# NVIDIA-Genomics-Research/GenomeWorks

Measured on AMD Instinct MI355X. Metric: cudapoa consensus GCUPS, 1024-window short-read batch (static band 256, 32 reads <= 1024 bp), higher is better.
Workload: dtype int16; 1 GPU; BASELINE configs[2]: cudapoa single-batch consensus, 1024 windows x 32 reads, backbone 960 bp, <=48 sub/24 ins/24 del, BatchConfig(1024,32,256,static_band), scores 8/-6/-8; windows_per_gpu=1024, cells_per_gpu=10990578176, parallelism=index-split x1

## Files before the change

### genomeworks_amd/csrc/gwhip_poa.hip

```cpp
#include <hip/hip_runtime.h>

#include <cstdio>
#include <cstdlib>
#include <cstring>
#include <string>

#include "poa_device.h"
#include "poa_full_device.h"
#include "poa_graph_device.h"
#include "poa_tb_device.h"

namespace gwhip
{

#ifndef GWHIP_POA_PART
thread_local std::string g_last_error;

static int fail(hipError_t e, const char* what)
{
    g_last_error = std::string(what) + ": " + hipGetErrorString(e);
    return (int)e;
}
static int fail_msg(int code, const std::string& msg)
{
    g_last_error = msg;
    return code;
}
#endif

constexpr int kRingBytes   = 8448;
constexpr int kRowInfoLds  = 3074;
constexpr int kRowInfoBytes = kRowInfoLds * 8;
constexpr int kReadLds     = 2048;
constexpr int kCodeTileLds = 4096;
static_assert(kReadLds + kCodeTileLds >= 3072 * 2, "the incremental topsort keeps the previous order (uint16 x 3072) in the read + code-tile regions");
constexpr int kBsRingBytes   = 2048;
constexpr int kReadWinBytes  = 4096;
constexpr int kMwLds         = 768;
constexpr size_t kReservedCuLds = 128 * 1024;

struct KernelArgs
{
    gwhip_poa_config cfg;
    PoaLayout L;
    int32_t total_windows;
    const uint8_t* sequences;
    const int8_t* base_weights;
    int32_t* sequence_lengths;
    const gwhip_window_details* window_details;
    uint8_t* consensus;
    uint16_t* coverage;
    uint8_t* msa;
    uint8_t* workspace;
    uint8_t* full_scores;
    uint64_t* cells;
    uint64_t* phase_cycles;
    int32_t debug_flags;
    int32_t cons_lds_nodes;
    int32_t wide_ring_bytes;
    uint32_t* work_counters;
};

// ... 2 lines not shown
{
    GraphView<IdT> g;
    g.nodes                = slab + L.nodes;
    g.incoming_edge_count  = (uint16_t*)(slab + L.in_cnt);
    g.outgoing_edge_count  = (uint16_t*)(slab + L.out_cnt);
    g.node_alignment_count = (uint16_t*)(slab + L.aln_cnt);
    g.coverage             = (uint16_t*)(slab + L.coverage);
    g.sorted_poa           = (IdT*)(slab + L.sorted);
    g.node_id_to_pos       = (IdT*)(slab + L.pos);
    g.local_cnt            = (uint16_t*)(slab + L.local_cnt);
    g.incoming_edges       = (IdT*)(slab + L.in_edges);
    g.incoming_edge_w      = (uint16_t*)(slab + L.in_w);
    g.outgoing_edges       = (IdT*)(slab + L.out_edges);
    g.node_alignments      = (IdT*)(slab + L.aligned);
    g.cons_scores          = (int32_t*)(slab + L.cons_scores);
    g.cons_pred            = (IdT*)(slab + L.cons_pred);
    g.marks                = slab + L.marks;
    g.check                = slab + L.check;
    g.to_visit             = (IdT*)(slab + L.to_visit);
    g.out_cov              = (uint16_t*)(slab + L.out_cov);
    g.out_cov_cnt          = (uint16_t*)(slab + L.out_cov_cnt);
    g.msa_pos              = (IdT*)(slab + L.msa_pos);
    g.seq_begin            = (IdT*)(slab + L.seq_begin);
    return g;
}

template <typename ScoreT, typename IdT, typename TraceT, int BM, bool MSA, bool LDS_TABLES, int NW, int VARIANT>
__global__ __launch_bounds__(kWave * NW) void poa_window_kernel(KernelArgs a)
{
    constexpr bool DBG = VARIANT == 1 || VARIANT == 4 || VARIANT == 6;
    constexpr int PV   = VARIANT == 0 ? 0 : (VARIANT <= 2 ? 1 : 2);
    constexpr bool kFullPacked = (VARIANT == 5 || VARIANT == 6) && BM == GWHIP_FULL_BAND && LDS_TABLES && std::is_same<ScoreT, int16_t>::value;
    const int32_t debug_flags = DBG ? a.debug_flags : 0;
    extern __shared__ __attribute__((aligned(16))) uint8_t smem[];
    const int lane       = threadIdx.x & (kWave - 1);
    const int wave       = __builtin_amdgcn_readfirstlane((int)threadIdx.x >> 6);
    for (int32_t w = blockIdx.x; w < a.total_windows;)
    {
    const gwhip_poa_config& c = a.cfg;
    uint8_t* slab        = a.workspace + (size_t)w * a.L.per_window;
    GraphView<IdT> g     = carve_graph<IdT>(slab, a.L);
    const gwhip_window_details wd = a.window_details[w];
    int32_t* seq_lens    = a.sequence_lengths + wd.seq_len_buffer_offset;
    const uint8_t* sequence    = a.sequences + wd.seq_starts;
    const int8_t* base_weights = a.base_weights + wd.seq_starts;
    uint8_t* consensus   = a.consensus + (size_t)w * c.max_consensus_size;
    int32_t* alignment_graph = (int32_t*)(slab + a.L.align_graph);
    int32_t* alignment_read  = (int32_t*)(slab + a.L.align_read);

    ScoreT* ring = reinterpret_cast<ScoreT*>(smem);
    uint8_t* lds_rowinfo_region = smem + kRingBytes;
    uint8_t* lds_read_buf       = smem + kRingBytes + kRowInfoBytes;
    uint8_t* lds_code_tile      = LDS_TABLES ? smem + kRingBytes + kRowInfoBytes + kReadLds : nullptr;
    const int32_t ring_bytes    = LDS_TABLES ? kRingBytes : a.wide_ring_bytes;
    int32_t* lds_bs_ring        = LDS_TABLES ? nullptr : reinterpret_cast<int32_t*>(smem + ring_bytes);
    uint8_t* lds_read_window    = LDS_TABLES ? nullptr : smem + ring_bytes + kBsRingBytes;
    uint8_t* codes              = a.L.codes ? slab + a.L.codes : nullptr;
    constexpr bool graph_fits_lds = LDS_TABLES;
    using RowT = RowInfo<LDS_TABLES>;
    RowT* rowinfo;
    if constexpr (LDS_TABLES)
        rowinfo = reinterpret_cast<RowT*>(smem + kRingBytes);
    else
        rowinfo = reinterpret_cast<RowT*>(slab + a.L.rowinfo);

    constexpr bool TB = (BM == GWHIP_STATIC_BAND_TRACEBACK || BM == GWHIP_ADAPTIVE_BAND_TRACEBACK);
    ScoreT* scores;
    uint8_t* full_moves = nullptr;
    if (BM == GWHIP_FULL_BAND)
    {
        const size_t cell_bytes = sizeof(ScoreT) + (sizeof(ScoreT) == 2 ? 1 : 0);
        uint8_t* region         = a.full_scores + (size_t)wd.scores_offset * (size_t)c.max_nodes_per_graph * cell_bytes;
        scores                  = reinterpret_cast<ScoreT*>(region);
        if (sizeof(ScoreT) == 2) full_moves = region + (size_t)wd.scores_width * (size_t)c.max_nodes_per_graph * sizeof(ScoreT);
    }
    else
        scores = reinterpret_cast<ScoreT*>(slab + a.L.scores);
    TraceT* traceback = TB ? reinterpret_cast<TraceT*>(slab + a.L.trace) : nullptr;
    const float banded_buffer_size = __fmul_rn((float)c.max_nodes_per_graph, (float)c.matrix_sequence_dimension);
    MwArgs<ScoreT>* mw_args = nullptr;
    MwShared* mw_shared     = nullptr;
    if constexpr (NW > 1)
    {
        {
            int32_t bases = lane < (int32_t)wd.num_seqs ? seq_lens[lane] : 0;
            for (int off = 32; off > 0; off >>= 1) bases += __shfl_xor(bases, off);
            bases = __builtin_amdgcn_readfirstlane(bases);
// ... 7 lines not shown
        mw_shared = reinterpret_cast<MwShared*>(smem + ring_bytes + kBsRingBytes + kReadWinBytes + 128);
        if (wave != 0)
        {
            for (;;)
            {
                block_barrier();
                const MwArgs<ScoreT> A = *mw_args;
                if (A.op != 1) return;
                generic_forward_skew<ScoreT, IdT, RowT, DBG>(A, g, rowinfo, ring, mw_shared, wave, lane);
            }
        }
    }

    const int32_t len0 = seq_lens[0];
    for (int32_t i = lane; i < len0; i += kWave)
    {
        g.nodes[i]                = sequence[i];
        g.sorted_poa[i]           = (IdT)i;
        g.node_id_to_pos[i]       = (IdT)i;
        g.node_alignment_count[i] = 0;
        g.coverage[i]             = 1;
        g.outgoing_edge_count[i]  = (i == len0 - 1) ? 0 : 1;
        g.local_cnt[i] = (uint16_t)(1 | ((i == len0 - 1 ? 0 : 1) << 4) | ((i == 0 ? 0 : 1) << 10));
        if (i < len0 - 1)
        {
            g.outgoing_edges[(int64_t)i * kEdges] = (IdT)(i + 1);
            if (MSA)
            {
                g.out_cov[(int64_t)i * kEdges * c.max_sequences_per_poa] = 0;
                g.out_cov_cnt[(int64_t)i * kEdges]                       = 1;
            }
        }
        if (i == 0)
        {
            g.incoming_edge_count[0] = 0;
            g.incoming_edge_w[0]     = (uint16_t)base_weights[0];
            if (MSA) g.seq_begin[0] = 0;
        }
        else
        {
            g.incoming_edges[(int64_t)i * kEdges]  = (IdT)(i - 1);
            g.incoming_edge_w[(int64_t)i * kEdges] = (uint16_t)(base_weights[i - 1] + base_weights[i]);
            g.incoming_edge_count[i]               = 1;
        }
    }
    if (lane == 0) consensus[0] = 0;
    uint64_t cells = 0;
    int32_t node_count = len0;
    uint64_t phase_acc[kPhCount] = {0, 0, 0, 0, 0, 0};
    PhaseClock pc{(DBG && a.phase_cycles) ? phase_acc : nullptr, 0};
    wave_sync();
    pc.start();

    for (int32_t s = 1; s < (int32_t)wd.num_seqs; s++)
    {
        const int32_t seq_len = seq_lens[s];
        const int32_t adv     = ((s == 1 ? len0 : seq_lens[s - 1]) + 3) & ~3;
        sequence += adv;
        base_weights += adv;

        if (node_count >= c.max_nodes_per_graph)
        {
            if (lane == 0) { consensus[0] = kKernelError; consensus[1] = kNodeCountExceeded; }
            break;
        }
        pc.tick(kPhOther);
        build_rowinfo<IdT, RowT>(g, node_count, rowinfo, lane, LDS_TABLES ? reinterpret_cast<uint64_t*>(lds_code_tile) : nullptr);
        constexpr bool LDS_READ = LDS_TABLES && BM != GWHIP_FULL_BAND;
        const uint8_t* lds_read = lds_read_buf;
        if constexpr (LDS_READ)
        {
            typedef uint32_t StageVec __attribute__((ext_vector_type(4)));
            typedef StageVec StageVecA4 __attribute__((aligned(4)));
            static_assert(kReadLds % 16 == 0 && (kRingBytes + kRowInfoBytes) % 16 == 0, "16-byte fetches fill the LDS copy of the read");
            const int32_t stage_bytes = min(kReadLds, ((max(seq_len, kMaxAdaptiveBand) + 8) + 3) & ~3);
            for (int32_t i = lane * 16; i < stage_bytes; i += kWave * 16)
                *reinterpret_cast<StageVec*>(lds_read_buf + i) = *reinterpret_cast<const StageVecA4*>(sequence + i);
        }
        wave_sync();
        pc.tick(kPhRowInfo);
        const uint8_t* banded_read = LDS_READ ? lds_read : sequence;

        int32_t alen = 0;
        constexpr bool kTbPacked = TB && LDS_TABLES && std::is_same<ScoreT, int16_t>::value && std::is_same<TraceT, int16_t>::value;
        bool tb_handled = false;
        if constexpr (kTbPacked)
        {
            constexpr bool kAd = BM == GWHIP_ADAPTIVE_BAND_TRACEBACK;
            const bool adaptive_now = kAd && c.alignment_band_width < kMaxAdaptiveBand;
            auto packed = [&](auto ad_tag, int32_t rerun) -> int32_t {
// ... 85 lines not shown
        {
            int32_t new_count   = 0;
            int32_t* scratch    = reinterpret_cast<int32_t*>(scores);
            const int32_t lpad  = (seq_len + 63) & ~63;
            par_rc = add_alignment_parallel<IdT, MSA, int32_t>(new_count, g, node_count, alen, alignment_graph, alignment_read,
                                                               sequence, base_weights, seq_len, MSA ? g.seq_begin + s : nullptr,
                                                               (uint16_t)s, (uint32_t)c.max_sequences_per_poa,
                                                               c.max_nodes_per_graph, scratch, scratch + lpad,
                                                               reinterpret_cast<uint32_t*>(scratch + 2 * lpad), lane,
                                                               debug_flags, pc.acc ? &pc.acc[kPhOther] : nullptr);
            if (par_rc == 0)
            {
                if (lane == 0) seq_lens[0] = new_count;
                status_and_count = new_count;
            }
            else if (par_rc > 0)
            {
                if (lane == 0) { consensus[0] = kKernelError; consensus[1] = (uint8_t)par_rc; }
                status_and_count = -1;
            }
        }
        const uint8_t* merge_read = (LDS_READ && !TB) ? lds_read : sequence;
        if constexpr (LDS_TABLES)
        {
            int32_t new_count = 0;
            par_rc = add_alignment_parallel<IdT, MSA>(new_count, g, node_count, alen, alignment_graph, alignment_read,
                                                      merge_read, base_weights, seq_len, MSA ? g.seq_begin + s : nullptr,
                                                      (uint16_t)s, (uint32_t)c.max_sequences_per_poa,
                                                      c.max_nodes_per_graph, reinterpret_cast<int16_t*>(smem),
                                                      reinterpret_cast<int16_t*>(smem) + 2048,
                                                      reinterpret_cast<uint32_t*>(lds_rowinfo_region), lane, debug_flags,
                                                      pc.acc ? &pc.acc[kPhOther] : nullptr);
            if (par_rc == 0)
            {
                if (lane == 0) seq_lens[0] = new_count;
                status_and_count = new_count;
            }
            else if (par_rc > 0)
            {
                if (lane == 0) { consensus[0] = kKernelError; consensus[1] = (uint8_t)par_rc; }
                status_and_count = -1;
            }
        }
        if (lane == 0 && par_rc < 0)
        {
            int32_t new_count = 0;
            uint8_t e = add_alignment_to_graph<IdT, MSA>(new_count, g, node_count, alen, alignment_graph, merge_read,
                                                         alignment_read, base_weights, MSA ? g.seq_begin + s : nullptr,
                                                         (uint16_t)s, (uint32_t)c.max_sequences_per_poa,
                                                         (uint32_t)c.max_nodes_per_graph);
            if (e != 0)
            {
                consensus[0]     = kKernelError;
                consensus[1]     = e;
                status_and_count = -1;
            }
            else
            {
                seq_lens[0]      = new_count;
                status_and_count = new_count;
            }
        }
        pc.tick(kPhAddAlignment);
        status_and_count = wave_first(status_and_count);
        constexpr bool kCachedSort = !LDS_TABLES && !TB && BM != GWHIP_FULL_BAND;
        bool sorted_here = false;
        if constexpr (kCachedSort)
        {
            const bool incr_ok = c.max_nodes_per_graph <= 131071 && !(debug_flags & (1 << 17)) &&
                                 (int64_t)a.L.scores_elems * (int64_t)sizeof(ScoreT) >= (int64_t)c.max_nodes_per_graph * 24 + 2048;
            if (status_and_count >= 0 && !c.spoa_accurate && !(debug_flags & (1 << 21)) && incr_ok)
            {
                wave_sync();
                bool done = false;
                if (!(debug_flags & (1 << 16)) && topsort_incr_cnt8_lds_bytes(status_and_count) <= ring_bytes)
                    done = topsort_kahn_incr_cnt8<IdT>(g, node_count, status_and_count, smem, reinterpret_cast<int32_t*>(scores), lane);
                if (!done) topsort_kahn_incr_hbm<IdT>(g, node_count, status_and_count, reinterpret_cast<int32_t*>(scores), lane);
                sorted_here = true;
            }
            else if (status_and_count >= 0 && !c.spoa_accurate && !(debug_flags & (1 << 21)) &&
                     (int64_t)a.L.scores_elems * (int64_t)sizeof(ScoreT) >= (int64_t)(2 * ((node_count + 63) & ~63)) * 4)
            {
                wave_sync();
                topsort_kahn_cached<IdT>(g, node_count, status_and_count, smem, reinterpret_cast<int32_t*>(scores), lane);
                sorted_here = true;
            }
        }
// ... 547 lines not shown
```

### genomeworks_amd/csrc/poa_device.h

```cpp
#pragma once
#include <hip/hip_runtime.h>
#include <stdint.h>

#include <type_traits>

#include "poa_layout.h"
#include "poa_pred_rows.h"

namespace gwhip
{

constexpr int kWave = 64;

template <typename T> struct Limits;
template <> struct Limits<int16_t> { static constexpr int32_t min = -32768; };
template <> struct Limits<int32_t> { static constexpr int32_t min = INT32_MIN; };

template <typename ScoreT> struct alignas(sizeof(ScoreT) * 4) Quad { ScoreT v[4]; };

template <typename ScoreT> __device__ __forceinline__ int32_t narrow_chk(int32_t v, bool& wrapped)
{
    const int32_t n = (int32_t)(ScoreT)v;
    if constexpr (sizeof(ScoreT) == 2) wrapped |= n != v;
    return n;
}

template <bool PACKED> struct RowInfo;
template <> struct alignas(8) RowInfo<true>
{
// ... 33 lines not shown
template <typename IdT> struct GraphView
{
    uint8_t* nodes;
    IdT* node_alignments;
    uint16_t* node_alignment_count;
    IdT* incoming_edges;
    uint16_t* incoming_edge_count;
    IdT* outgoing_edges;
    uint16_t* outgoing_edge_count;
    uint16_t* incoming_edge_w;
    IdT* sorted_poa;
    IdT* node_id_to_pos;
    uint16_t* local_cnt;
    uint16_t* coverage;
    int32_t* cons_scores;
    IdT* cons_pred;
    uint8_t* marks;
    uint8_t* check;
    IdT* to_visit;
    uint16_t* out_cov;
    uint16_t* out_cov_cnt;
    IdT* msa_pos;
    IdT* seq_begin;
};

__device__ __forceinline__ int32_t band_start_for_row(int32_t row, float gradient, int32_t band_width,
                                                      int32_t band_shift, int32_t max_column)
{
    int32_t diagonal_index = (int32_t)(__fmul_rn((float)row, gradient));
    int32_t start_pos      = max(0, diagonal_index - band_shift);
    if (max_column < start_pos + band_width) start_pos = max(0, max_column - band_width + kCellsPerLane);
    start_pos = start_pos - (start_pos % kCellsPerLane);
    return start_pos;
}

enum Phase { kPhRowInfo = 0, kPhForward, kPhTraceback, kPhAddAlignment, kPhTopsort, kPhOther, kPhCount };
struct PhaseClock
{
    uint64_t* acc;
    uint64_t last;
    __device__ void start() { if (acc) last = clock64(); }
    __device__ void tick(int phase)
    {
        if (acc)
        {
            uint64_t now = clock64();
// ... 611 lines not shown
    const uint64_t t_pp = psel == 6 ? clock64() : 0;
    if (aligned_nodes > 0 && (aligned_nodes & (kStage - 1)) != 0)
        flush_stage(aligned_nodes & ~(kStage - 1), aligned_nodes & (kStage - 1));
    if ((dbg & 2) && prof_acc && lane == 0) *prof_acc += (uint64_t)max(aligned_nodes, 0);
    if (aligned_nodes >= bound) aligned_nodes = kNwLoopFailed;
    wave_sync();
    for (int32_t k0 = lane; k0 < aligned_nodes; k0 += 4 * kWave)
    {
        int32_t pos[4], node[4];
#pragma unroll
        for (int u = 0; u < 4; u++) pos[u] = (k0 + u * kWave < aligned_nodes) ? alignment_graph[k0 + u * kWave] : -1;
#pragma unroll
        for (int u = 0; u < 4; u++) node[u] = (int32_t)g.sorted_poa[max(pos[u], 0)];
#pragma unroll
        for (int u = 0; u < 4; u++)
            if (pos[u] >= 0) alignment_graph[k0 + u * kWave] = node[u];
    }
    wave_sync();
    if (psel == 6) pacc += clock64() - t_pp;
    if (psel && lane == 0) *prof_acc += pacc;
    return aligned_nodes;
}

template <typename IdT, typename RowT>
__device__ __forceinline__ void build_rowinfo(const GraphView<IdT>& g, int32_t graph_count, RowT* rowinfo, int lane,
                                              uint64_t* xpred = nullptr)
{
    if (xpred != nullptr)
    {
#pragma unroll
        for (int q = 0; q < 4; q++) xpred[q * kWave + lane] = 0;
        wave_sync();
    }
    if (lane == 0) rowinfo[0].set(0, 0, false, 0, 0, 0);
    constexpr int kU = 4;
    for (int32_t r0 = 1 + lane; r0 <= graph_count; r0 += kU * kWave)
    {
        int32_t node[kU], cnt[kU], oc[kU], bas[kU], e0[kU], e1[kU], e2[kU], q0[kU], q1[kU], q2[kU];
        int32_t e3[kU], e4[kU], e5[kU], q3[kU] = {}, q4[kU] = {}, q5[kU] = {};
#pragma unroll
        for (int u = 0; u < kU; u++) node[u] = g.sorted_poa[min(r0 + u * kWave, graph_count) - 1];
#pragma unroll
        for (int u = 0; u < kU; u++)
        {
            cnt[u] = g.incoming_edge_count[node[u]];
            oc[u]  = g.outgoing_edge_count[node[u]];
            bas[u] = g.nodes[node[u]];
            e0[u]  = g.incoming_edges[(int64_t)node[u] * kEdges + 0];
            e1[u]  = g.incoming_edges[(int64_t)node[u] * kEdges + 1];
            e2[u]  = g.incoming_edges[(int64_t)node[u] * kEdges + 2];
        }
#pragma unroll
        for (int u = 0; u < kU; u++)
        {
            q0[u] = g.node_id_to_pos[(uint32_t)e0[u] < (uint32_t)graph_count ? e0[u] : 0];
            q1[u] = g.node_id_to_pos[(uint32_t)e1[u] < (uint32_t)graph_count ? e1[u] : 0];
            q2[u] = g.node_id_to_pos[(uint32_t)e2[u] < (uint32_t)graph_count ? e2[u] : 0];
            e3[u] = e4[u] = e5[u] = 0;
            if (xpred != nullptr && cnt[u] > 3)
            {
                e3[u] = g.incoming_edges[(int64_t)node[u] * kEdges + 3];
                e4[u] = g.incoming_edges[(int64_t)node[u] * kEdges + 4];
                e5[u] = g.incoming_edges[(int64_t)node[u] * kEdges + 5];
            }
        }
        if (xpred != nullptr)
        {
            bool any = false;
#pragma unroll
            for (int u = 0; u < kU; u++) any |= cnt[u] > 3;
            if (__ballot(any) != 0)
            {
#pragma unroll
                for (int u = 0; u < kU; u++)
                {
                    q3[u] = q4[u] = q5[u] = 0;
                    if (cnt[u] > 3)
                    {
                        q3[u] = g.node_id_to_pos[(uint32_t)e3[u] < (uint32_t)graph_count ? e3[u] : 0];
                        q4[u] = g.node_id_to_pos[(uint32_t)e4[u] < (uint32_t)graph_count ? e4[u] : 0];
                        q5[u] = g.node_id_to_pos[(uint32_t)e5[u] < (uint32_t)graph_count ? e5[u] : 0];
                    }
                }
            }
        }
#pragma unroll
        for (int u = 0; u < kU; u++)
        {
            const int32_t r = r0 + u * kWave;
            if (r <= graph_count)
            {
                RowT ri{};
                ri.set(bas[u], cnt[u], oc[u] == 0, cnt[u] > 0 ? q0[u] + 1 : 0, cnt[u] > 1 ? q1[u] + 1 : 0, cnt[u] > 2 ? q2[u] + 1 : 0);
                rowinfo[r] = ri;
                if (xpred != nullptr && cnt[u] > 3)
                    xpred[r & (kSideTableSlots - 1)] = xpred_entry(r, cnt[u], q3[u] + 1, q4[u] + 1, q5[u] + 1);
            }
        }
    }
}

template <typename ScoreT, typename IdT>
__device__ __forceinline__ void banded_forward_1pass(const GraphView<IdT>& g, const RowInfo<true>* rowinfo,
                                                     int32_t graph_count, const uint8_t* lds_read, ScoreT* scores,
// ... 1348 lines not shown
```

### genomeworks_amd/csrc/poa_graph_device.h

```cpp
#pragma once
#include "poa_device.h"

namespace gwhip
{

template <typename IdT, bool MSA>
__device__ uint8_t add_alignment_to_graph(int32_t& new_node_count, const GraphView<IdT>& g, int32_t node_count,
                                          int32_t alignment_length, const int32_t* alignment_graph,
                                          const uint8_t* read, const int32_t* alignment_read,
                                          const int8_t* base_weights, IdT* sequence_begin_nodes_ids, uint16_t s,
                                          uint32_t max_sequences_per_poa, uint32_t max_limit_nodes_per_window)
{
    int32_t head_node_id = -1;
    int32_t curr_node_id = -1;
    uint16_t prev_weight = 0;
    for (int32_t pos = alignment_length - 1; pos >= 0; pos--)
    {
        int32_t read_pos = alignment_read[pos];
        if (read_pos == -1) continue;
        int8_t node_weight    = base_weights[read_pos];
        uint8_t read_base     = read[read_pos];
        int32_t graph_node_id = alignment_graph[pos];
        if (graph_node_id == -1)
        {
            curr_node_id = node_count++;
            if ((uint32_t)node_count >= max_limit_nodes_per_window) return kNodeCountExceeded;
            g.nodes[curr_node_id]                = read_base;
            g.outgoing_edge_count[curr_node_id]  = 0;
            g.incoming_edge_count[curr_node_id]  = 0;
            g.node_alignment_count[curr_node_id] = 0;
            g.coverage[curr_node_id]             = 0;
        }
        else
        {
            uint8_t graph_base = g.nodes[graph_node_id];
            if (graph_base == read_base)
                curr_node_id = graph_node_id;
            else
            {
                uint16_t num_aligned    = g.node_alignment_count[graph_node_id];
                int32_t aligned_node_id = -1;
                for (int32_t n = 0; n < num_aligned; n++)
                {
                    int32_t aid = g.node_alignments[(int64_t)graph_node_id * kAligns + n];
                    if (g.nodes[aid] == read_base)
                    {
                        aligned_node_id = aid;
                        break;
                    }
                }
                if (aligned_node_id != -1)
                    curr_node_id = aligned_node_id;
                else
                {
                    curr_node_id = node_count++;
                    if ((uint32_t)node_count >= max_limit_nodes_per_window) return kNodeCountExceeded;
                    g.nodes[curr_node_id]                = read_base;
                    g.outgoing_edge_count[curr_node_id]  = 0;
                    g.incoming_edge_count[curr_node_id]  = 0;
                    g.node_alignment_count[curr_node_id] = 0;
                    g.coverage[curr_node_id]             = 0;
                    int32_t new_alignments               = 0;
                    for (int32_t n = 0; n < num_aligned; n++)
                    {
                        int32_t aid        = g.node_alignments[(int64_t)graph_node_id * kAligns + n];
                        uint16_t aid_count = g.node_alignment_count[aid];
                        g.node_alignments[(int64_t)aid * kAligns + aid_count]               = (IdT)curr_node_id;
                        g.node_alignment_count[aid]                                         = aid_count + 1;
                        g.node_alignments[(int64_t)curr_node_id * kAligns + new_alignments] = (IdT)aid;
                        new_alignments++;
                    }
                    g.node_alignments[(int64_t)graph_node_id * kAligns + num_aligned]   = (IdT)curr_node_id;
                    g.node_alignment_count[graph_node_id]                               = num_aligned + 1;
                    g.node_alignments[(int64_t)curr_node_id * kAligns + new_alignments] = (IdT)graph_node_id;
                    new_alignments++;
                    g.node_alignment_count[curr_node_id] = (uint16_t)new_alignments;
                }
            }
        }
        if (MSA && read_pos == 0) *sequence_begin_nodes_ids = (IdT)curr_node_id;
        if (head_node_id != -1)
        {
            bool edge_exists  = false;
            uint16_t in_count = g.incoming_edge_count[curr_node_id];
            for (int32_t e = 0; e < in_count; e++)
            {
                if (g.incoming_edges[(int64_t)curr_node_id * kEdges + e] == head_node_id)
                {
                    edge_exists = true;
                    g.incoming_edge_w[(int64_t)curr_node_id * kEdges + e] += (uint16_t)(prev_weight + node_weight);
                }
            }
            if (!edge_exists)
            {
                g.incoming_edges[(int64_t)curr_node_id * kEdges + in_count]  = (IdT)head_node_id;
                g.incoming_edge_w[(int64_t)curr_node_id * kEdges + in_count] = (uint16_t)(prev_weight + node_weight);
                g.incoming_edge_count[curr_node_id]                          = in_count + 1;
                uint16_t out_count                                           = g.outgoing_edge_count[head_node_id];
                g.outgoing_edges[(int64_t)head_node_id * kEdges + out_count] = (IdT)curr_node_id;
                if (MSA)
                {
                    g.out_cov_cnt[(int64_t)head_node_id * kEdges + out_count] = 1;
                    g.out_cov[((int64_t)head_node_id * kEdges + out_count) * max_sequences_per_poa] = s;
                }
                g.outgoing_edge_count[head_node_id] = out_count + 1;
                if (out_count + 1 >= kEdges || in_count + 1 >= kEdges) return kEdgeCountExceeded;
            }
            else if (MSA)
            {
                uint16_t out_count = g.outgoing_edge_count[head_node_id];
                for (int32_t e = 0; e < out_count; e++)
                {
                    if (g.outgoing_edges[(int64_t)head_node_id * kEdges + e] == curr_node_id)
                    {
                        uint16_t cc = g.out_cov_cnt[(int64_t)head_node_id * kEdges + e];
                        g.out_cov[((int64_t)head_node_id * kEdges + e) * max_sequences_per_poa + cc] = s;
                        g.out_cov_cnt[(int64_t)head_node_id * kEdges + e]                            = cc + 1;
                        break;
                    }
                }
            }
        }
        head_node_id = curr_node_id;
        g.coverage[head_node_id]++;
        prev_weight = (uint16_t)node_weight;
    }
    new_node_count = node_count;
    return 0;
}

template <typename IdT, bool MSA, typename NodeT = int16_t>
__device__ __forceinline__ int32_t add_alignment_parallel(int32_t& new_node_count, const GraphView<IdT>& g,
                                                          int32_t node_count, int32_t alen, const int32_t* ag,
                                                          const int32_t* ar, const uint8_t* read,
                                                          const int8_t* base_weights, int32_t read_length,
                                                          IdT* sequence_begin_nodes_ids, uint16_t s,
                                                          uint32_t max_sequences_per_poa, int32_t max_nodes,
                                                          NodeT* gnode, NodeT* curr, uint32_t* onpath, int lane,
                                                          int32_t dbg = 0, uint64_t* prof_acc = nullptr)
{
    const int32_t L = read_length;
    const int32_t prof_sel = (dbg >> 16) & 7;
    uint64_t prof_t = prof_sel ? clock64() : 0;
    auto prof_mark = [&](int32_t which) {
        if (prof_sel)
        {
            const uint64_t now = clock64();
            if (prof_sel == which && prof_acc) *prof_acc += now - prof_t;
            prof_t = now;
        }
    };
    for (int32_t i = lane; i < (node_count + 31) / 32; i += kWave) onpath[i] = 0;
    for (int32_t i = lane; i < L; i += kWave) gnode[i] = -1;
    wave_sync();
// ... 96 lines not shown
        int32_t rp_edgeerr = INT32_MAX;
        for (int32_t rp = 1 + lane; rp < rp_nodeerr; rp += kWave)
        {
            const int32_t head = curr[rp - 1], cur = curr[rp];
            const int32_t ic   = in_count_of(cur);
            bool exists        = false;
            for (int32_t e = 0; e < ic; e++)
                if (g.incoming_edges[(int64_t)cur * kEdges + e] == head) exists = true;
            if (!exists && (out_count_of(head) + 1 >= kEdges || ic + 1 >= kEdges)) rp_edgeerr = min(rp_edgeerr, rp);
        }
        for (int off = 32; off > 0; off >>= 1) rp_edgeerr = min(rp_edgeerr, __shfl_xor(rp_edgeerr, off));
        return rp_edgeerr != INT32_MAX ? (int32_t)kEdgeCountExceeded : (int32_t)kNodeCountExceeded;
    }

    for (int32_t rp = lane; rp < L; rp += kWave)
    {
        const int32_t cur = curr[rp];
        if (cur < first_new) continue;
        const int32_t gn          = gnode[rp];
        g.nodes[cur]               = read[rp];
        g.outgoing_edge_count[cur] = 0;
        g.incoming_edge_count[cur] = 0;
        g.coverage[cur]            = 0;
        int32_t na_new             = 0;
        if (gn >= 0)
        {
            const int32_t na = g.node_alignment_count[gn];
            for (int32_t n = 0; n < na; n++)
            {
                const int32_t aid  = g.node_alignments[(int64_t)gn * kAligns + n];
                const int32_t acnt = g.node_alignment_count[aid];
                g.node_alignments[(int64_t)aid * kAligns + acnt] = (IdT)cur;
                g.node_alignment_count[aid]                      = (uint16_t)(acnt + 1);
                g.node_alignments[(int64_t)cur * kAligns + n]    = (IdT)aid;
            }
            g.node_alignments[(int64_t)gn * kAligns + na]  = (IdT)cur;
            g.node_alignment_count[gn]                     = (uint16_t)(na + 1);
            g.node_alignments[(int64_t)cur * kAligns + na] = (IdT)gn;
            na_new                                         = na + 1;
        }
        g.node_alignment_count[cur] = (uint16_t)na_new;
    }
    wave_sync();
    prof_mark(3);

    int32_t rp_edgeerr = INT32_MAX;
    constexpr int kUD = 4, kBatch = 4;
    for (int32_t rp0 = lane; rp0 < L; rp0 += kUD * kWave)
    {
        int32_t cur[kUD], head[kUD], ic[kUD], oc_head[kUD], be[kUD][kBatch];
        uint16_t cov[kUD], w[kUD], bw[kUD][kBatch];
#pragma unroll
        for (int u = 0; u < kUD; u++)
        {
            const int32_t rp = min(rp0 + u * kWave, L - 1);
            cur[u]  = curr[rp];
            head[u] = rp > 0 ? (int32_t)curr[rp - 1] : cur[u];
            w[u]    = rp > 0 ? (uint16_t)((uint16_t)base_weights[rp - 1] + base_weights[rp]) : (uint16_t)0;
        }
#pragma unroll
        for (int u = 0; u < kUD; u++)
        {
            cov[u]     = g.coverage[cur[u]];
            ic[u]      = in_count_of(cur[u]);
            oc_head[u] = out_count_of(head[u]);
#pragma unroll
            for (int e = 0; e < kBatch; e++)
            {
                be[u][e] = g.incoming_edges[(int64_t)cur[u] * kEdges + e];
                bw[u][e] = g.incoming_edge_w[(int64_t)cur[u] * kEdges + e];
            }
        }
#pragma unroll
        for (int u = 0; u < kUD; u++)
        {
            const int32_t rp = rp0 + u * kWave;
            if (rp >= L) continue;
            if (rp > 0)
            {
                bool exists = false;
#pragma unroll
                for (int e = 0; e < kBatch; e++)
                    if (e < ic[u] && be[u][e] == head[u])
                    {
                        exists = true;
                        g.incoming_edge_w[(int64_t)cur[u] * kEdges + e] = (uint16_t)(bw[u][e] + w[u]);
                    }
                for (int32_t e = kBatch; e < ic[u]; e++)
                {
                    if (g.incoming_edges[(int64_t)cur[u] * kEdges + e] == head[u])
                    {
                        exists = true;
                        g.incoming_edge_w[(int64_t)cur[u] * kEdges + e] += w[u];
                    }
                }
                if (!exists)
                {
                    g.incoming_edges[(int64_t)cur[u] * kEdges + ic[u]]  = (IdT)head[u];
                    g.incoming_edge_w[(int64_t)cur[u] * kEdges + ic[u]] = w[u];
                    g.incoming_edge_count[cur[u]]                       = (uint16_t)(ic[u] + 1);
                    const int32_t oc                                    = oc_head[u];
                    g.outgoing_edges[(int64_t)head[u] * kEdges + oc]    = (IdT)cur[u];
                    if (MSA)
                    {
                        g.out_cov_cnt[(int64_t)head[u] * kEdges + oc]                       = 1;
                        g.out_cov[((int64_t)head[u] * kEdges + oc) * max_sequences_per_poa] = s;
                    }
                    g.outgoing_edge_count[head[u]] = (uint16_t)(oc + 1);
                    if (oc + 1 >= kEdges || ic[u] + 1 >= kEdges) rp_edgeerr = min(rp_edgeerr, rp);
                }
                else if (MSA)
                {
                    const int32_t oc = oc_head[u];
                    for (int32_t e = 0; e < oc; e++)
                    {
                        if (g.outgoing_edges[(int64_t)head[u] * kEdges + e] == cur[u])
                        {
                            const uint16_t cc = g.out_cov_cnt[(int64_t)head[u] * kEdges + e];
                            g.out_cov[((int64_t)head[u] * kEdges + e) * max_sequences_per_poa + cc] = s;
                            g.out_cov_cnt[(int64_t)head[u] * kEdges + e]                            = cc + 1;
                            break;
                        }
                    }
                }
            }
            else if (MSA)
                *sequence_begin_nodes_ids = (IdT)cur[u];
            g.coverage[cur[u]] = (uint16_t)(cov[u] + 1);
        }
    }
    for (int off = 32; off > 0; off >>= 1) rp_edgeerr = min(rp_edgeerr, __shfl_xor(rp_edgeerr, off));
    wave_sync();
    prof_mark(4);
    if (rp_edgeerr != INT32_MAX) return (int32_t)kEdgeCountExceeded;
    new_node_count = node_count + running;
    return 0;
}

template <typename IdT>
__device__ void topsort_kahn(IdT* sorted_poa, IdT* node_map, int32_t node_count, const uint16_t* incoming_edge_count,
                             const IdT* outgoing_edges, const uint16_t* outgoing_edge_count, uint16_t* local_cnt)
{
    int32_t position = 0;
    for (int32_t n = 0; n < node_count; n++)
    {
        uint16_t c   = incoming_edge_count[n];
        local_cnt[n] = c;
        if (c == 0)
        {
            node_map[n]            = (IdT)position;
            sorted_poa[position++] = (IdT)n;
        }
    }
    for (int32_t n = 0; n < position; n++)
    {
        int32_t node = sorted_poa[n];
        uint16_t oc  = outgoing_edge_count[node];
        for (int32_t e = 0; e < oc; e++)
        {
// ... 244 lines not shown
{
    const int32_t tsel = prof_acc ? (dbg >> 25) & 7 : 0;
    uint64_t tacc      = 0;
    const uint64_t t_p1 = tsel == 1 ? clock64() : 0;
    constexpr int32_t kDummy = 3073;
    constexpr int32_t kQClip = 15;
    uint64_t* ent   = reinterpret_cast<uint64_t*>(lds);
    uint32_t* ent32 = reinterpret_cast<uint32_t*>(lds);
    uint16_t* queue = reinterpret_cast<uint16_t*>(lds_queue);
    uint16_t* sold  = reinterpret_cast<uint16_t*>(lds_old);
    uint64_t* wide  = reinterpret_cast<uint64_t*>(lds_queue + 6144 + 16);
    auto hi_of = [&](int32_t n) -> uint32_t { return ent32[2 * n + 1]; };
    auto wide_hit = [&](uint64_t we, int32_t n) -> bool {
        return (int32_t)(we & 0xfffu) == n && ((we >> 12) & 1u) != 0 && ((we >> 13) & 63u) <= 6u;
    };
#pragma unroll
    for (int q = 0; q < 4; q++) wide[q * kWave + lane] = 0;
    wave_sync();
    int32_t tail = 0;
    constexpr int kU = 4;
    for (int32_t base = 0; base < node_count; base += kU * kWave)
    {
        uint32_t ic[kU], oc[kU], e0[kU], e1[kU], e2[kU], e3[kU], e4[kU], e5[kU], m[kU], po[kU], so[kU];
#pragma unroll
        for (int u = 0; u < kU; u++)
        {
            const int32_t n  = min(base + u * kWave + lane, node_count - 1);
            const int32_t nn = n >= n_old ? 0 : n;
            ic[u] = g.incoming_edge_count[n];
            oc[u] = g.outgoing_edge_count[n];
            e0[u] = (uint32_t)g.outgoing_edges[(int64_t)n * kEdges] & 0xfffu;
            e1[u] = (uint32_t)g.outgoing_edges[(int64_t)n * kEdges + 1] & 0xfffu;
            e2[u] = (uint32_t)g.outgoing_edges[(int64_t)n * kEdges + 2] & 0xfffu;
            e3[u] = (uint32_t)g.outgoing_edges[(int64_t)n * kEdges + 3] & 0xfffu;
            e4[u] = (uint32_t)g.outgoing_edges[(int64_t)n * kEdges + 4] & 0xfffu;
            e5[u] = (uint32_t)g.outgoing_edges[(int64_t)n * kEdges + 5] & 0xfffu;
            m[u]  = g.local_cnt[nn];
            po[u] = (uint32_t)g.node_id_to_pos[nn] & 0xfffu;
            so[u] = (uint32_t)g.sorted_poa[nn] & 0xfffu;
        }
#pragma unroll
        for (int u = 0; u < kU; u++)
        {
            const int32_t n = base + u * kWave + lane;
            bool is_src     = false;
            if (n < node_count)
            {
                const bool is_new = n >= n_old;
                if (!is_new) sold[n] = (uint16_t)so[u];
                const uint32_t din  = (is_new || ((m[u] >> 10) & 63u) != ic[u]) ? 1u : 0u;
                const uint32_t dout = (is_new || ((m[u] >> 4) & 63u) != oc[u]) ? 1u : 0u;
                const uint32_t lo   = (oc[u] > 0 ? e0[u] : 0u) | (oc[u] > 1 ? e1[u] << 12 : 0u) | (min(oc[u], 4u) << 24) |
                                    (is_new ? 0u : (m[u] & 15u) << 27);
                const uint32_t hi = (ic[u] & 0x3fu) | (din << 6) | (dout << 7) | (is_new ? 0u : po[u] << 8) | (oc[u] > 2 ? e2[u] << 20 : 0u);
                ent[n] = (uint64_t)lo | ((uint64_t)hi << 32);
                if (oc[u] > 3)
                    wide[n & 255] = (uint64_t)((uint32_t)n | (1u << 12) | (oc[u] << 13) | (e3[u] << 20)) | ((uint64_t)e4[u] << 32) |
                                    ((uint64_t)e5[u] << 44);
                is_src = (ic[u] == 0);
            }
            const unsigned long long ms = __ballot(is_src);
            if (is_src) queue[tail + __popcll(ms & ((1ull << lane) - 1))] = (uint16_t)n;
// ... 1156 lines not shown
```

Measured before the change: 454.8 GCUPS.

## Add packed 16-byte node heads to gather graph adjacency in single loads

Adds a packed per-node header (base, in-degree, first three incoming edges; out-degree, first four outgoing edges) kept in the slab's unused row-table region and updated by both merge paths. The row-info builder and the incremental topological sort now read one 16-byte header per node instead of many scattered count and edge loads, falling back to the full edge arrays only for high-degree nodes. This cuts scattered global memory traffic in the graph-maintenance phases. In exchange, every edge insertion does extra header writes, and a debug-only consistency checker plus a serial-merge debug flag are added.

After: 453.6 GCUPS. About the same (-0.3%).

```diff
diff --git a/genomeworks_amd/csrc/gwhip_poa.hip b/genomeworks_amd/csrc/gwhip_poa.hip
--- a/genomeworks_amd/csrc/gwhip_poa.hip
+++ b/genomeworks_amd/csrc/gwhip_poa.hip
@@ -38,6 +38,9 @@
 constexpr int kReadWinBytes  = 4096;
 constexpr int kMwLds         = 768;
 constexpr size_t kReservedCuLds = 128 * 1024;
+
+constexpr int32_t kDbgHeadCheck   = 1 << 19;
+constexpr int32_t kDbgSerialMerge = INT32_MIN;
 
 struct KernelArgs
 {
@@ -86,6 +89,7 @@
     g.out_cov_cnt          = (uint16_t*)(slab + L.out_cov_cnt);
     g.msa_pos              = (IdT*)(slab + L.msa_pos);
     g.seq_begin            = (IdT*)(slab + L.seq_begin);
+    g.heads                = nullptr;
     return g;
 }
 
@@ -127,6 +131,9 @@
         rowinfo = reinterpret_cast<RowT*>(smem + kRingBytes);
     else
         rowinfo = reinterpret_cast<RowT*>(slab + a.L.rowinfo);
+    constexpr bool HEADS = LDS_TABLES;
+    static_assert(sizeof(NodeHead) == 16 && sizeof(NodeHead) <= sizeof(RowInfo<false>), "the heads fit the row-table region of the slab");
+    if constexpr (HEADS) g.heads = reinterpret_cast<NodeHead*>(slab + a.L.rowinfo);
 
     constexpr bool TB = (BM == GWHIP_STATIC_BAND_TRACEBACK || BM == GWHIP_ADAPTIVE_BAND_TRACEBACK);
     ScoreT* scores;
@@ -180,6 +187,8 @@
         g.coverage[i]             = 1;
         g.outgoing_edge_count[i]  = (i == len0 - 1) ? 0 : 1;
         g.local_cnt[i] = (uint16_t)(1 | ((i == len0 - 1 ? 0 : 1) << 4) | ((i == 0 ? 0 : 1) << 10));
+        if constexpr (HEADS)
+            g.heads[i] = NodeHead{head_in_pack(sequence[i], i == 0 ? 0 : 1, i - 1, 0, 0), head_out_pack(i == len0 - 1 ? 0 : 1, i + 1, 0, 0, 0)};
         if (i < len0 - 1)
         {
             g.outgoing_edges[(int64_t)i * kEdges] = (IdT)(i + 1);
@@ -223,7 +232,7 @@
             break;
         }
         pc.tick(kPhOther);
-        build_rowinfo<IdT, RowT>(g, node_count, rowinfo, lane, LDS_TABLES ? reinterpret_cast<uint64_t*>(lds_code_tile) : nullptr);
+        build_rowinfo<IdT, RowT, HEADS>(g, node_count, rowinfo, lane, LDS_TABLES ? reinterpret_cast<uint64_t*>(lds_code_tile) : nullptr);
         constexpr bool LDS_READ = LDS_TABLES && BM != GWHIP_FULL_BAND;
         const uint8_t* lds_read = lds_read_buf;
         if constexpr (LDS_READ)
@@ -355,9 +364,10 @@
         }
         const uint8_t* merge_read = (LDS_READ && !TB) ? lds_read : sequence;
         if constexpr (LDS_TABLES)
+        if (!(debug_flags & kDbgSerialMerge))
         {
             int32_t new_count = 0;
-            par_rc = add_alignment_parallel<IdT, MSA>(new_count, g, node_count, alen, alignment_graph, alignment_read,
+            par_rc = add_alignment_parallel<IdT, MSA, int16_t, HEADS>(new_count, g, node_count, alen, alignment_graph, alignment_read,
                                                       merge_read, base_weights, seq_len, MSA ? g.seq_begin + s : nullptr,
                                                       (uint16_t)s, (uint32_t)c.max_sequences_per_poa,
                                                       c.max_nodes_per_graph, reinterpret_cast<int16_t*>(smem),
@@ -378,7 +388,7 @@
         if (lane == 0 && par_rc < 0)
         {
             int32_t new_count = 0;
-            uint8_t e = add_alignment_to_graph<IdT, MSA>(new_count, g, node_count, alen, alignment_graph, merge_read,
+            uint8_t e = add_alignment_to_graph<IdT, MSA, HEADS>(new_count, g, node_count, alen, alignment_graph, merge_read,
                                                          alignment_read, base_weights, MSA ? g.seq_begin + s : nullptr,
                                                          (uint16_t)s, (uint32_t)c.max_sequences_per_poa,
                                                          (uint32_t)c.max_nodes_per_graph);
@@ -396,6 +406,16 @@
         }
         pc.tick(kPhAddAlignment);
         status_and_count = wave_first(status_and_count);
+        if constexpr (HEADS && DBG)
+        {
+            if ((debug_flags & kDbgHeadCheck) && !(debug_flags & (1 << 14)) && status_and_count >= 0 && pc.acc)
+            {
+                wave_sync();
+                const int32_t bad  = check_node_heads<IdT>(g, status_and_count, lane);
+                const int32_t room = 4095 - (int32_t)(pc.acc[kPhOther] >> 52);
+                pc.acc[kPhOther] += ((uint64_t)(uint32_t)status_and_count << 32) + ((uint64_t)min(bad, room) << 52);
+            }
+        }
         constexpr bool kCachedSort = !LDS_TABLES && !TB && BM != GWHIP_FULL_BAND;
         bool sorted_here = false;
         if constexpr (kCachedSort)
diff --git a/genomeworks_amd/csrc/poa_device.h b/genomeworks_amd/csrc/poa_device.h
--- a/genomeworks_amd/csrc/poa_device.h
+++ b/genomeworks_amd/csrc/poa_device.h
@@ -5,6 +5,7 @@
 #include <type_traits>
 
 #include "poa_layout.h"
+#include "poa_node_heads.h"
 #include "poa_pred_rows.h"
 
 namespace gwhip
@@ -84,6 +85,7 @@
     uint16_t* out_cov_cnt;
     IdT* msa_pos;
     IdT* seq_begin;
+    NodeHead* heads;
 };
 
 __device__ __forceinline__ int32_t band_start_for_row(int32_t row, float gradient, int32_t band_width,
@@ -741,7 +743,7 @@
     return aligned_nodes;
 }
 
-template <typename IdT, typename RowT>
+template <typename IdT, typename RowT, bool HEADS = false>
 __device__ __forceinline__ void build_rowinfo(const GraphView<IdT>& g, int32_t graph_count, RowT* rowinfo, int lane,
                                               uint64_t* xpred = nullptr)
 {
@@ -757,48 +759,115 @@
     {
         int32_t node[kU], cnt[kU], oc[kU], bas[kU], e0[kU], e1[kU], e2[kU], q0[kU], q1[kU], q2[kU];
         int32_t e3[kU], e4[kU], e5[kU], q3[kU] = {}, q4[kU] = {}, q5[kU] = {};
+        uint64_t hin[kU] = {};
 #pragma unroll
         for (int u = 0; u < kU; u++) node[u] = g.sorted_poa[min(r0 + u * kWave, graph_count) - 1];
 #pragma unroll
         for (int u = 0; u < kU; u++)
         {
-            cnt[u] = g.incoming_edge_count[node[u]];
-            oc[u]  = g.outgoing_edge_count[node[u]];
-            bas[u] = g.nodes[node[u]];
-            e0[u]  = g.incoming_edges[(int64_t)node[u] * kEdges + 0];
-            e1[u]  = g.incoming_edges[(int64_t)node[u] * kEdges + 1];
-            e2[u]  = g.incoming_edges[(int64_t)node[u] * kEdges + 2];
-        }
-#pragma unroll
-        for (int u = 0; u < kU; u++)
-        {
-            q0[u] = g.node_id_to_pos[(uint32_t)e0[u] < (uint32_t)graph_count ? e0[u] : 0];
-            q1[u] = g.node_id_to_pos[(uint32_t)e1[u] < (uint32_t)graph_count ? e1[u] : 0];
-            q2[u] = g.node_id_to_pos[(uint32_t)e2[u] < (uint32_t)graph_count ? e2[u] : 0];
-            e3[u] = e4[u] = e5[u] = 0;
-            if (xpred != nullptr && cnt[u] > 3)
-            {
-                e3[u] = g.incoming_edges[(int64_t)node[u] * kEdges + 3];
-                e4[u] = g.incoming_edges[(int64_t)node[u] * kEdges + 4];
-                e5[u] = g.incoming_edges[(int64_t)node[u] * kEdges + 5];
-            }
-        }
-        if (xpred != nullptr)
+            if constexpr (HEADS)
+            {
+                const NodeHead hd = g.heads[node[u]];
+                hin[u] = hd.in;
+                oc[u]  = (int32_t)(uint32_t)hd.out;
+            }
+            else
+            {
+                cnt[u] = g.incoming_edge_count[node[u]];
+                oc[u]  = g.outgoing_edge_count[node[u]];
+                bas[u] = g.nodes[node[u]];
+                e0[u]  = g.incoming_edges[(int64_t)node[u] * kEdges + 0];
+                e1[u]  = g.incoming_edges[(int64_t)node[u] * kEdges + 1];
+                e2[u]  = g.incoming_edges[(int64_t)node[u] * kEdges + 2];
+            }
+        }
+        if constexpr (HEADS)
+        {
+            asm volatile("" : "+v"(hin[0]), "+v"(hin[1]), "+v"(hin[2]), "+v"(hin[3]), "+v"(oc[0]), "+v"(oc[1]), "+v"(oc[2]), "+v"(oc[3]));
+#pragma unroll
+            for (int u = 0; u < kU; u++)
+            {
+                cnt[u] = head_in_degree(hin[u]);
+                oc[u]  = head_out_degree((uint64_t)(uint32_t)oc[u]);
+                bas[u] = head_base(hin[u]);
+                e0[u]  = head_in_edge(hin[u], 0);
+                e1[u]  = head_in_edge(hin[u], 1);
+                e2[u]  = head_in_edge(hin[u], 2);
+            }
+        }
+        if constexpr (HEADS)
         {
             bool any = false;
 #pragma unroll
-            for (int u = 0; u < kU; u++) any |= cnt[u] > 3;
-            if (__ballot(any) != 0)
+            for (int u = 0; u < kU; u++)
+            {
+                q0[u] = g.node_id_to_pos[(uint32_t)e0[u] < (uint32_t)graph_count ? e0[u] : 0];
+                q1[u] = g.node_id_to_pos[(uint32_t)e1[u] < (uint32_t)graph_count ? e1[u] : 0];
+                q2[u] = g.node_id_to_pos[(uint32_t)e2[u] < (uint32_t)graph_count ? e2[u] : 0];
+                e3[u] = e4[u] = e5[u] = 0;
+                any |= cnt[u] > 3;
+            }
+            const bool wide = xpred != nullptr && __ballot(any) != 0;
+            if (wide)
             {
 #pragma unroll
                 for (int u = 0; u < kU; u++)
                 {
-                    q3[u] = q4[u] = q5[u] = 0;
-                    if (cnt[u] > 3)
+                    const int64_t at = (int64_t)(cnt[u] > 3 ? node[u] : 0) * kEdges;
+                    e3[u] = g.incoming_edges[at + 3];
+                    e4[u] = g.incoming_edges[at + 4];
+                    e5[u] = g.incoming_edges[at + 5];
+                }
+            }
+            asm volatile("" : "+v"(q0[0]), "+v"(q0[1]), "+v"(q0[2]), "+v"(q0[3]), "+v"(q1[0]), "+v"(q1[1]), "+v"(q1[2]), "+v"(q1[3]),
+                              "+v"(q2[0]), "+v"(q2[1]), "+v"(q2[2]), "+v"(q2[3]), "+v"(e3[0]), "+v"(e3[1]), "+v"(e3[2]), "+v"(e3[3]),
+                              "+v"(e4[0]), "+v"(e4[1]), "+v"(e4[2]), "+v"(e4[3]), "+v"(e5[0]), "+v"(e5[1]), "+v"(e5[2]), "+v"(e5[3]));
+            if (wide)
+            {
+#pragma unroll
+                for (int u = 0; u < kU; u++)
+                {
+                    q3[u] = g.node_id_to_pos[(cnt[u] > 3 && (uint32_t)e3[u] < (uint32_t)graph_count) ? e3[u] : 0];
+                    q4[u] = g.node_id_to_pos[(cnt[u] > 3 && (uint32_t)e4[u] < (uint32_t)graph_count) ? e4[u] : 0];
+                    q5[u] = g.node_id_to_pos[(cnt[u] > 3 && (uint32_t)e5[u] < (uint32_t)graph_count) ? e5[u] : 0];
+                }
+                asm volatile("" : "+v"(q3[0]), "+v"(q3[1]), "+v"(q3[2]), "+v"(q3[3]), "+v"(q4[0]), "+v"(q4[1]), "+v"(q4[2]), "+v"(q4[3]),
+                                  "+v"(q5[0]), "+v"(q5[1]), "+v"(q5[2]), "+v"(q5[3]));
+            }
+        }
+        else
+        {
+#pragma unroll
+            for (int u = 0; u < kU; u++)
+            {
+                q0[u] = g.node_id_to_pos[(uint32_t)e0[u] < (uint32_t)graph_count ? e0[u] : 0];
+                q1[u] = g.node_id_to_pos[(uint32_t)e1[u] < (uint32_t)graph_count ? e1[u] : 0];
+                q2[u] = g.node_id_to_pos[(uint32_t)e2[u] < (uint32_t)graph_count ? e2[u] : 0];
+                e3[u] = e4[u] = e5[u] = 0;
+                if (xpred != nullptr && cnt[u] > 3)
+                {
+                    e3[u] = g.incoming_edges[(int64_t)node[u] * kEdges + 3];
+                    e4[u] = g.incoming_edges[(int64_t)node[u] * kEdges + 4];
+                    e5[u] = g.incoming_edges[(int64_t)node[u] * kEdges + 5];
+                }
+            }
+            if (xpred != nullptr)
+            {
+                bool any = false;
+#pragma unroll
+                for (int u = 0; u < kU; u++) any |= cnt[u] > 3;
+                if (__ballot(any) != 0)
+                {
+#pragma unroll
+                    for (int u = 0; u < kU; u++)
                     {
-                        q3[u] = g.node_id_to_pos[(uint32_t)e3[u] < (uint32_t)graph_count ? e3[u] : 0];
-                        q4[u] = g.node_id_to_pos[(uint32_t)e4[u] < (uint32_t)graph_count ? e4[u] : 0];
-                        q5[u] = g.node_id_to_pos[(uint32_t)e5[u] < (uint32_t)graph_count ? e5[u] : 0];
+                        q3[u] = q4[u] = q5[u] = 0;
+                        if (cnt[u] > 3)
+                        {
+                            q3[u] = g.node_id_to_pos[(uint32_t)e3[u] < (uint32_t)graph_count ? e3[u] : 0];
+                            q4[u] = g.node_id_to_pos[(uint32_t)e4[u] < (uint32_t)graph_count ? e4[u] : 0];
+                            q5[u] = g.node_id_to_pos[(uint32_t)e5[u] < (uint32_t)graph_count ? e5[u] : 0];
+                        }
                     }
                 }
             }
diff --git a/genomeworks_amd/csrc/poa_graph_device.h b/genomeworks_amd/csrc/poa_graph_device.h
--- a/genomeworks_amd/csrc/poa_graph_device.h
+++ b/genomeworks_amd/csrc/poa_graph_device.h
@@ -4,7 +4,7 @@
 namespace gwhip
 {
 
-template <typename IdT, bool MSA>
+template <typename IdT, bool MSA, bool HEADS = false>
 __device__ uint8_t add_alignment_to_graph(int32_t& new_node_count, const GraphView<IdT>& g, int32_t node_count,
                                           int32_t alignment_length, const int32_t* alignment_graph,
                                           const uint8_t* read, const int32_t* alignment_read,
@@ -30,6 +30,7 @@
             g.incoming_edge_count[curr_node_id]  = 0;
             g.node_alignment_count[curr_node_id] = 0;
             g.coverage[curr_node_id]             = 0;
+            if constexpr (HEADS) g.heads[curr_node_id] = NodeHead{head_in_new(read_base), head_out_new()};
         }
         else
         {
@@ -60,6 +61,7 @@
                     g.incoming_edge_count[curr_node_id]  = 0;
                     g.node_alignment_count[curr_node_id] = 0;
                     g.coverage[curr_node_id]             = 0;
+                    if constexpr (HEADS) g.heads[curr_node_id] = NodeHead{head_in_new(read_base), head_out_new()};
                     int32_t new_alignments               = 0;
                     for (int32_t n = 0; n < num_aligned; n++)
                     {
@@ -104,6 +106,11 @@
                     g.out_cov[((int64_t)head_node_id * kEdges + out_count) * max_sequences_per_poa] = s;
                 }
                 g.outgoing_edge_count[head_node_id] = out_count + 1;
+                if constexpr (HEADS)
+                {
+                    g.heads[curr_node_id].in  = head_in_append(g.heads[curr_node_id].in, head_node_id);
+                    g.heads[head_node_id].out = head_out_append(g.heads[head_node_id].out, curr_node_id);
+                }
                 if (out_count + 1 >= kEdges || in_count + 1 >= kEdges) return kEdgeCountExceeded;
             }
             else if (MSA)
@@ -129,7 +136,7 @@
     return 0;
 }
 
-template <typename IdT, bool MSA, typename NodeT = int16_t>
+template <typename IdT, bool MSA, typename NodeT = int16_t, bool HEADS = false>
 __device__ __forceinline__ int32_t add_alignment_parallel(int32_t& new_node_count, const GraphView<IdT>& g,
                                                           int32_t node_count, int32_t alen, const int32_t* ag,
                                                           const int32_t* ar, const uint8_t* read,
@@ -272,6 +279,7 @@
         g.outgoing_edge_count[cur] = 0;
         g.incoming_edge_count[cur] = 0;
         g.coverage[cur]            = 0;
+        if constexpr (HEADS) g.heads[cur] = NodeHead{head_in_new(read[rp]), head_out_new()};
         int32_t na_new             = 0;
         if (gn >= 0)
         {
@@ -300,6 +308,7 @@
     {
         int32_t cur[kUD], head[kUD], ic[kUD], oc_head[kUD], be[kUD][kBatch];
         uint16_t cov[kUD], w[kUD], bw[kUD][kBatch];
+        uint64_t hd_out[kUD] = {};
 #pragma unroll
         for (int u = 0; u < kUD; u++)
         {
@@ -313,13 +322,21 @@
         {
             cov[u]     = g.coverage[cur[u]];
             ic[u]      = in_count_of(cur[u]);
-            oc_head[u] = out_count_of(head[u]);
+            if constexpr (HEADS)
+                hd_out[u] = g.heads[head[u]].out;
+            else
+                oc_head[u] = out_count_of(head[u]);
 #pragma unroll
             for (int e = 0; e < kBatch; e++)
             {
                 be[u][e] = g.incoming_edges[(int64_t)cur[u] * kEdges + e];
                 bw[u][e] = g.incoming_edge_w[(int64_t)cur[u] * kEdges + e];
             }
+        }
+        if constexpr (HEADS)
+        {
+#pragma unroll
+            for (int u = 0; u < kUD; u++) oc_head[u] = head_out_degree(hd_out[u]);
         }
 #pragma unroll
         for (int u = 0; u < kUD; u++)
@@ -357,6 +374,12 @@
                         g.out_cov[((int64_t)head[u] * kEdges + oc) * max_sequences_per_poa] = s;
                     }
                     g.outgoing_edge_count[head[u]] = (uint16_t)(oc + 1);
+                    if constexpr (HEADS)
+                    {
+                        g.heads[cur[u]].in = head_in_pack(read[rp], ic[u] + 1, ic[u] == 0 ? head[u] : be[u][0], ic[u] == 1 ? head[u] : be[u][1],
+                                                          ic[u] == 2 ? head[u] : be[u][2]);
+                        g.heads[head[u]].out = head_out_append(hd_out[u], cur[u]);
+                    }
                     if (oc + 1 >= kEdges || ic[u] + 1 >= kEdges) rp_edgeerr = min(rp_edgeerr, rp);
                 }
                 else if (MSA)
@@ -385,6 +408,29 @@
     if (rp_edgeerr != INT32_MAX) return (int32_t)kEdgeCountExceeded;
     new_node_count = node_count + running;
     return 0;
+}
+
+template <typename IdT>
+__device__ int32_t check_node_heads(const GraphView<IdT>& g, int32_t node_count, int lane)
+{
+    int32_t bad = 0;
+    for (int32_t n0 = 0; n0 < node_count; n0 += kWave)
+    {
+        const int32_t n = n0 + lane;
+        bool differs    = false;
+        if (n < node_count)
+        {
+            const int32_t ic = g.incoming_edge_count[n], oc = g.outgoing_edge_count[n];
+            const IdT* ie    = g.incoming_edges + (int64_t)n * kEdges;
+            const IdT* oe    = g.outgoing_edges + (int64_t)n * kEdges;
+            const uint64_t in  = head_in_pack(g.nodes[n], ic, ic > 0 ? ie[0] : 0, ic > 1 ? ie[1] : 0, ic > 2 ? ie[2] : 0);
+            const uint64_t out = head_out_pack(oc, oc > 0 ? oe[0] : 0, oc > 1 ? oe[1] : 0, oc > 2 ? oe[2] : 0, oc > 3 ? oe[3] : 0);
+            const NodeHead hd  = g.heads[n];
+            differs            = hd.in != in || hd.out != out;
+        }
+        bad += __popcll(__ballot(differs));
+    }
+    return bad;
 }
 
 template <typename IdT>
@@ -675,22 +721,55 @@
     for (int32_t base = 0; base < node_count; base += kU * kWave)
     {
         uint32_t ic[kU], oc[kU], e0[kU], e1[kU], e2[kU], e3[kU], e4[kU], e5[kU], m[kU], po[kU], so[kU];
+        uint64_t hin[kU] = {}, hout[kU] = {};
 #pragma unroll
         for (int u = 0; u < kU; u++)
         {
             const int32_t n  = min(base + u * kWave + lane, node_count - 1);
             const int32_t nn = n >= n_old ? 0 : n;
-            ic[u] = g.incoming_edge_count[n];
-            oc[u] = g.outgoing_edge_count[n];
-            e0[u] = (uint32_t)g.outgoing_edges[(int64_t)n * kEdges] & 0xfffu;
-            e1[u] = (uint32_t)g.outgoing_edges[(int64_t)n * kEdges + 1] & 0xfffu;
-            e2[u] = (uint32_t)g.outgoing_edges[(int64_t)n * kEdges + 2] & 0xfffu;
-            e3[u] = (uint32_t)g.outgoing_edges[(int64_t)n * kEdges + 3] & 0xfffu;
-            e4[u] = (uint32_t)g.outgoing_edges[(int64_t)n * kEdges + 4] & 0xfffu;
-            e5[u] = (uint32_t)g.outgoing_edges[(int64_t)n * kEdges + 5] & 0xfffu;
-            m[u]  = g.local_cnt[nn];
-            po[u] = (uint32_t)g.node_id_to_pos[nn] & 0xfffu;
-            so[u] = (uint32_t)g.sorted_poa[nn] & 0xfffu;
+            const NodeHead hd = g.heads[n];
+            hin[u]  = hd.in;
+            hout[u] = hd.out;
+            m[u]    = g.local_cnt[nn];
+            po[u]   = (uint32_t)g.node_id_to_pos[nn];
+            so[u]   = (uint32_t)g.sorted_poa[nn];
+        }
+        {
+            asm volatile("" : "+v"(hin[0]), "+v"(hin[1]), "+v"(hin[2]), "+v"(hin[3]), "+v"(hout[0]), "+v"(hout[1]), "+v"(hout[2]), "+v"(hout[3]),
+                              "+v"(m[0]), "+v"(m[1]), "+v"(m[2]), "+v"(m[3]), "+v"(po[0]), "+v"(po[1]), "+v"(po[2]), "+v"(po[3]),
+                              "+v"(so[0]), "+v"(so[1]), "+v"(so[2]), "+v"(so[3]));
+            bool more = false;
+#pragma unroll
+            for (int u = 0; u < kU; u++)
+            {
+                ic[u] = (uint32_t)head_in_degree(hin[u]);
+                oc[u] = (uint32_t)head_out_degree(hout[u]);
+                e0[u] = (uint32_t)head_out_edge(hout[u], 0);
+                e1[u] = (uint32_t)head_out_edge(hout[u], 1);
+                e2[u] = (uint32_t)head_out_edge(hout[u], 2);
+                e3[u] = (uint32_t)head_out_edge(hout[u], 3);
+                e4[u] = e5[u] = 0;
+                po[u] &= 0xfffu;
+                so[u] &= 0xfffu;
+                more |= oc[u] > 4u;
+            }
+            if (__ballot(more) != 0)
+            {
+#pragma unroll
+                for (int u = 0; u < kU; u++)
+                {
+                    const int32_t n = oc[u] > 4u ? min(base + u * kWave + lane, node_count - 1) : 0;
+                    e4[u] = (uint32_t)g.outgoing_edges[(int64_t)n * kEdges + 4];
+                    e5[u] = (uint32_t)g.outgoing_edges[(int64_t)n * kEdges + 5];
+                }
+                asm volatile("" : "+v"(e4[0]), "+v"(e4[1]), "+v"(e4[2]), "+v"(e4[3]), "+v"(e5[0]), "+v"(e5[1]), "+v"(e5[2]), "+v"(e5[3]));
+#pragma unroll
+                for (int u = 0; u < kU; u++)
+                {
+                    e4[u] = oc[u] > 4u ? e4[u] & 0xfffu : 0u;
+                    e5[u] = oc[u] > 4u ? e5[u] & 0xfffu : 0u;
+                }
+            }
         }
 #pragma unroll
         for (int u = 0; u < kU; u++)
diff --git a/genomeworks_amd/csrc/poa_node_heads.h b/genomeworks_amd/csrc/poa_node_heads.h
--- /dev/null
+++ b/genomeworks_amd/csrc/poa_node_heads.h
@@ -0,0 +1,54 @@
+#pragma once
+
+#include <cstdint>
+
+#if defined(__HIPCC__)
+#define GWHIP_NODE_HEADS_FN __host__ __device__ inline
+#else
+#define GWHIP_NODE_HEADS_FN inline
+#endif
+
+namespace gwhip
+{
+
+constexpr int kHeadInEdges  = 3;
+constexpr int kHeadOutEdges = 4;
+
+struct alignas(16) NodeHead
+{
+    uint64_t in;
+    uint64_t out;
+};
+
+GWHIP_NODE_HEADS_FN uint64_t head_in_new(int32_t base) { return (uint64_t)(base & 0xff); }
+GWHIP_NODE_HEADS_FN int32_t head_base(uint64_t in) { return (int32_t)(in & 0xffu); }
+GWHIP_NODE_HEADS_FN int32_t head_in_degree(uint64_t in) { return (int32_t)((in >> 8) & 0x3fu); }
+GWHIP_NODE_HEADS_FN int32_t head_in_edge(uint64_t in, int32_t k) { return (int32_t)((in >> (14 + 12 * k)) & 0xfffu); }
+GWHIP_NODE_HEADS_FN uint64_t head_in_pack(int32_t base, int32_t degree, int32_t e0, int32_t e1, int32_t e2)
+{
+    return (uint64_t)(base & 0xff) | ((uint64_t)(degree & 0x3f) << 8) | (degree > 0 ? (uint64_t)(e0 & 0xfff) << 14 : 0) |
+           (degree > 1 ? (uint64_t)(e1 & 0xfff) << 26 : 0) | (degree > 2 ? (uint64_t)(e2 & 0xfff) << 38 : 0);
+}
+GWHIP_NODE_HEADS_FN uint64_t head_in_append(uint64_t in, int32_t edge)
+{
+    const int32_t d = head_in_degree(in);
+    if (d < kHeadInEdges) in |= (uint64_t)(edge & 0xfff) << (14 + 12 * d);
+    return (in & ~((uint64_t)0x3f << 8)) | ((uint64_t)((d + 1) & 0x3f) << 8);
+}
+
+GWHIP_NODE_HEADS_FN uint64_t head_out_new() { return 0; }
+GWHIP_NODE_HEADS_FN int32_t head_out_degree(uint64_t out) { return (int32_t)(out & 0x3fu); }
+GWHIP_NODE_HEADS_FN int32_t head_out_edge(uint64_t out, int32_t k) { return (int32_t)((out >> (6 + 12 * k)) & 0xfffu); }
+GWHIP_NODE_HEADS_FN uint64_t head_out_pack(int32_t degree, int32_t e0, int32_t e1, int32_t e2, int32_t e3)
+{
+    return (uint64_t)(degree & 0x3f) | (degree > 0 ? (uint64_t)(e0 & 0xfff) << 6 : 0) | (degree > 1 ? (uint64_t)(e1 & 0xfff) << 18 : 0) |
+           (degree > 2 ? (uint64_t)(e2 & 0xfff) << 30 : 0) | (degree > 3 ? (uint64_t)(e3 & 0xfff) << 42 : 0);
+}
+GWHIP_NODE_HEADS_FN uint64_t head_out_append(uint64_t out, int32_t edge)
+{
+    const int32_t d = head_out_degree(out);
+    if (d < kHeadOutEdges) out |= (uint64_t)(edge & 0xfff) << (6 + 12 * d);
+    return (out & ~(uint64_t)0x3f) | (uint64_t)((d + 1) & 0x3f);
+}
+
+}
```
